# zgspose/PAVENet

Measured on AMD Instinct MI355X. Metric: clips/sec (T=7, 800x1344) fwd, higher is better.
Workload: dtype f32 (exact 3-term bf16 split on the bf16 MFMA)

## Files before the change

include/pave_hip.h:

```cpp
#ifndef PAVE_HIP_H_
#define PAVE_HIP_H_

#include <stdint.h>

#ifdef __cplusplus
extern "C" {
#endif

#define PAVE_OK 0
#define PAVE_E_ARG (-1)
#define PAVE_E_LAUNCH (-2)
#define PAVE_E_STEP (-3)
#define PAVE_E_UNSUPPORTED (-4)

#define PAVE_ABI_VERSION 21
int pave_abi_version(void);
const char* pave_last_error(void);

int pave_ms_deform_attn_forward_f32(const float* value, const int64_t* spatial_shapes,
                                    const int64_t* level_start, const float* sampling_loc,
                                    const float* attn_weight, float* out, int bs, int S, int M,
                                    int D, int L, int Lq, int P, int im2col_step, void* stream);
int pave_ms_deform_attn_forward_f64(const double* value, const int64_t* spatial_shapes,
                                    const int64_t* level_start, const double* sampling_loc,
// ... 648 lines not shown
                                 float* out, long long M, int K, int N, int group_n, int relu,
                                 int nplanes, void* stream);

int pave_gemm_bf16x3_ln_f32(const float* a, const void* w_planes, const float* bias,
                            const float* residual, const float* gamma, const float* beta, float eps,
                            float* out, long long M, int K, int N, int nplanes, void* stream);

int pave_conv3x3_split_f32(const float* x, const void* w_planes, const float* bias,
                           const float* residual, float* y, int N, int H, int W, int Cin, int Cout,
                           int stride, int relu, int nplanes, void* stream);

long long pave_conv3x3_splitk_workspace_bytes(int N, int H, int W, int Cin, int Cout, int stride);
int pave_conv3x3_splitk_f32(const float* x, const void* w_planes, const float* bias,
                            const float* residual, float* y, int N, int H, int W, int Cin, int Cout,
                            int stride, int relu, void* workspace, long long workspace_bytes,
                            int nplanes, void* stream);

long long pave_gemm_splitk_workspace_bytes(long long M, int K, int N);
int pave_gemm_bf16x3_splitk_f32(const float* a, const void* w_planes, const float* bias, const float* residual,
                                float* out, long long M, int K, int N, int relu, int nplanes, void* workspace,
                                long long workspace_bytes, void* stream);

int pave_set_form_policy(int policy);
int pave_get_form_policy(void);

#define PAVE_FORM_ROWS 0
#define PAVE_FORM_ROWS_SPLITK 1
#define PAVE_FORM_ROWS_TILE 2
#define PAVE_FORM_LN 3
#define PAVE_FORM_CONV3X3 4
#define PAVE_FORM_CONV1X1S 5
#define PAVE_FORM_ENCPROJ 6
#define PAVE_ORDER_TILE 0
#define PAVE_ORDER_KSPLIT 1
#define PAVE_ORDER_SPLITK 2
#define PAVE_ORDER_TILE_LNPASS 3
#define PAVE_ORDER_KSPLIT_LNPASS 4
#define PAVE_ORDER_TILE_LN8 5
int pave_form_plan(long long M, int K, int N, int kind, int nplanes, int policy, int* order, int* ksplit);

int pave_bottleneck_chain_f32(const float* c1, const void* w2_planes, const float* b2, float* c2,
                              const void* w3_planes, const float* b3, const float* residual,
                              const float* a2, int k2, float* out, const void* w1n_planes,
                              const float* b1n, float* c1n, int cn, int N, int H, int W, int nplanes,
                              void* stream);

int pave_conv1x1_strided_split_f32(const float* x, const void* w_planes, const float* bias, float* y,
                                   int N, int H, int W, int Cin, int Cout, int stride, int relu,
                                   int nplanes, void* stream);

int pave_conv7x7s2_nchw_split_f32(const float* x, const void* w_planes, const float* bias, float* y,
                                  int N, int H, int W, int row_pitch, int Cout, int relu, int nplanes,
                                  void* stream);

int pave_repitch_rows_f32(const float* src, float* dst, long long rows, int W, int pitch, void* stream);

int pave_swin_window_attn_f32(const float* qkv, const float* bias_t, const float* pad_qkv, float* out, int B,
                              int H, int W, int C, int heads, int window, int shift, float scale, void* stream);

int pave_merge_softmax_partials_f32(const float* parts, float* out, int G, int U, int C, int H, void* stream);

int pave_split_bf16x3_f32(const float* x, void* planes, long long n, int nplanes, void* stream);

#define PAVE_AUG_MAX_AUGS 16
#define PAVE_AUG_MAX_SLOTS 128
#define PAVE_AUG_MAX_K 64
typedef struct pave_aug_plan {
  const float* bboxes[PAVE_AUG_MAX_AUGS];
  const float* kpts[PAVE_AUG_MAX_AUGS];
  const int32_t* keep[PAVE_AUG_MAX_AUGS];
  int32_t flip[PAVE_AUG_MAX_AUGS];
  float img_w[PAVE_AUG_MAX_SLOTS];
  float scale_factor[PAVE_AUG_MAX_SLOTS][4];
  int32_t flip_perm[PAVE_AUG_MAX_K];
  int32_t n_aug, B, N, K;
} pave_aug_plan;
int pave_aug_merge_nms_f32(const pave_aug_plan* plan, float score_thr, int max_num, int method, float iou_thr,
                           float sigma, float min_score, int offset, float* dets, int64_t* labels, float* kpts,
                           int64_t* inds, int32_t* keep, int32_t* count, void* stream);

int pave_hflip_canvas_f32(const float* x, float* y, const int32_t* valid_w, int valid_w_all, int n, int C, int Hp,
                          int Wp, void* stream);

#ifdef __cplusplus
}
#endif
#endif
```

pavenet_amd/build_native.py:

```python
import os
import subprocess
import sysconfig

_HERE = os.path.dirname(os.path.abspath(__file__))
ROOT = os.path.dirname(_HERE)
SOURCES = [os.path.join(_HERE, 'csrc', 'pave_kernels.hip'),
           os.path.join(_HERE, 'csrc', 'pave_gemm_split.hip'),
           os.path.join(_HERE, 'csrc', 'pave_enc_tile.hip'),
           os.path.join(_HERE, 'csrc', 'pave_gemm_dma.hip'),
           os.path.join(_HERE, 'csrc', 'pave_decoder.hip'),
           os.path.join(_HERE, 'csrc', 'pave_aug.hip'),
           os.path.join(_HERE, 'csrc', 'pave_ingest.hip'),
           os.path.join(_HERE, 'csrc', 'pave_draw.hip'),
           os.path.join(_HERE, 'csrc', 'pave_track.hip'),
           os.path.join(_HERE, 'csrc', 'pave_smooth.hip'),
           os.path.join(_HERE, 'csrc', 'pave_zones.hip'),
           os.path.join(_HERE, 'csrc', 'pave_posture.hip'),
           os.path.join(_HERE, 'csrc', 'pave_overlay.hip'),
           os.path.join(_HERE, 'csrc', 'pave_heat.hip'),
           os.path.join(_HERE, 'csrc', 'pave_trails.hip'),
           os.path.join(_HERE, 'csrc', 'pave_floor.hip'),
           os.path.join(_HERE, 'csrc', 'pave_contacts.hip'),
           os.path.join(_HERE, 'csrc', 'pave_reid.hip'),
           os.path.join(_HERE, 'csrc', 'pave_anon.hip')]
HEADERS = sorted(os.path.join(_HERE, 'csrc', f) for f in os.listdir(os.path.join(_HERE, 'csrc')) if f.endswith('.h')) + \
          [os.path.join(ROOT, 'include', 'pave_hip.h')]
OUT = os.path.join(_HERE, 'lib', 'libpave_hip.so')
OUT_DIAG = os.path.join(_HERE, 'lib', 'libpave_hip_diag.so')
EXT_SOURCE = os.path.join(_HERE, 'csrc', 'pave_mmcv_ext.cpp')
EXT_OUT = os.path.join(_HERE, '_ext' + (sysconfig.get_config_var('EXT_SUFFIX') or '.so'))


def _fresh(out, deps):
    return os.path.exists(out) and all(os.path.getmtime(out) >= os.path.getmtime(s) for s in deps)


def build_native(force=False, verbose=False, diag=True):
    os.makedirs(os.path.dirname(OUT), exist_ok=True)
    flavours = [('', [], OUT)] + ([('_diag', ['-DPAVE_DIAG=1'], OUT_DIAG)] if diag else [])
    hipcc = os.environ.get('HIPCC', '/opt/rocm/bin/hipcc')
    procs, links = [], []
    for suffix, defs, out in flavours:
        if not force and _fresh(out, SOURCES + HEADERS):
            continue
        objs = []
        for src in SOURCES:
            obj = os.path.join(_HERE, 'lib', os.path.basename(src).replace('.hip', suffix + '.o'))
            objs.append(obj)
            if not force and _fresh(obj, [src] + HEADERS):
                continue
            cmd = [hipcc, '-O3', '--offload-arch=gfx950', '-std=c++17', '-fPIC', '-c'] + defs + \
                  ['-I' + os.path.join(ROOT, 'include'), '-o', obj, src]
            if verbose and not suffix:
                cmd.insert(1, '-Rpass-analysis=kernel-resource-usage')
            procs.append((cmd, subprocess.Popen(cmd)))
        links.append((out, objs))
    for cmd, p in procs:
        if p.wait() != 0:
            raise subprocess.CalledProcessError(p.returncode, cmd)
    for out, objs in links:
        subprocess.check_call([hipcc, '--offload-arch=gfx950', '-shared', '-fPIC', '-o', out] + objs)
    return OUT


def build_ext(force=False):
    if not force and _fresh(EXT_OUT, [EXT_SOURCE, OUT] + HEADERS):
        return EXT_OUT
    import torch
    from torch.utils.cpp_extension import include_paths, library_paths
    cmd = ['g++', '-O2', '-std=c++17', '-shared', '-fPIC', '-D__HIP_PLATFORM_AMD__=1', '-DUSE_ROCM=1',
           '-DTORCH_EXTENSION_NAME=_ext', '-DTORCH_API_INCLUDE_EXTENSION_H',
           f'-D_GLIBCXX_USE_CXX11_ABI={int(torch._C._GLIBCXX_USE_CXX11_ABI)}',
           '-I/opt/rocm/include', '-I' + os.path.join(ROOT, 'include'),
           '-I' + sysconfig.get_paths()['include']] + ['-I' + p for p in include_paths()] + \
          [EXT_SOURCE, '-o', EXT_OUT, '-L' + os.path.dirname(OUT), '-lpave_hip',
           '-Wl,-rpath,$ORIGIN/lib'] + \
          [a for p in library_paths() for a in ('-L' + p, '-Wl,-rpath,' + p)] + \
          ['-lc10', '-lc10_hip', '-ltorch_cpu', '-ltorch_hip', '-ltorch', '-ltorch_python']
    subprocess.check_call(cmd)
    return EXT_OUT


if __name__ == '__main__':
    print(build_native(force=True, verbose=True))
    print(build_ext(force=True))
```

pavenet_amd/deform_attn.py:

```python
import math
import warnings

import torch
import torch.nn as nn

from . import ops
from .bricks import (BaseModule, SourceKey, batch_first, constant_init, linear_residual_norm,
                     linear_rows, seq_first_view, xavier_init)
from .census import note_slow_path
from .registry import ATTENTION, MMCV_ATTENTION


def frame_prefixes(num_frames):
    assert num_frames % 2 == 1, 'num_frames must be odd (centre frame + symmetric neighbours)'
    c = num_frames // 2
    return ['pre_' * (c - t) if t < c else 'next_' * (t - c) for t in range(num_frames)]


def _check_heads(embed_dims, num_heads):
    if embed_dims % num_heads != 0:
        raise ValueError(f'embed_dims must be divisible by num_heads, '
                         f'but got {embed_dims} and {num_heads}')
    d = embed_dims // num_heads
    if not (isinstance(d, int) and d > 0 and (d & (d - 1)) == 0):
# ... 3 lines not shown


class _CatProj:

    def _cat_sources(self):
        raise NotImplementedError

    def _cat_proj(self, frames=None):
        offs, logits = self._cat_sources()
        if frames is not None:
            offs, logits = [offs[t] for t in frames], [logits[t] for t in frames]
        srcs = [m.weight for m in offs + logits] + [m.bias for m in offs + logits]
        key = SourceKey(srcs, frames)
        if getattr(self, '_cat_key', None) != key:
            with torch.no_grad():
                self._cat_w = torch.cat([m.weight for m in offs + logits], 0).contiguous()
                self._cat_b = torch.cat([m.bias for m in offs + logits], 0).contiguous()
            self._cat_key = key
        return self._cat_w, self._cat_b


FOLD_QUERY_POS = True


def cat_proj_rows(mod, query, query_pos, frames=None):
    from .bricks import fold_pos_ok, fused_mode
    q = batch_first(query)
    bs, Q, C = q.shape
    pos_rows = None
    if (FOLD_QUERY_POS and query_pos is not None and q.is_cuda and q.dtype == torch.float32 and fused_mode()
            and not torch.is_grad_enabled() and query_pos.shape == query.shape and C % 64 == 0 and q.is_contiguous()):
        pb = query_pos.transpose(0, 1)
        if fold_pos_ok(pb, bs) and pb.stride(2) == 1:
            pos_rows = pb[0]
    if pos_rows is None:
        w, b = mod._cat_proj(frames)
        if query_pos is not None:
            q = batch_first(query + query_pos)
        return linear_rows(q.reshape(bs * Q, C), w, b)
    w, b = mod._cat_proj(frames)
    base = pos_rows._base if pos_rows._base is not None else pos_rows
    from .bricks import get_gemm_mode
    key = SourceKey((base, w, b), extra=(tuple(pos_rows.shape), tuple(pos_rows.stride()), pos_rows.storage_offset(),
                                        frames, get_gemm_mode()))
    hit = mod.__dict__.get('_pave_pos_proj')
    if hit is None or hit[0] != key:
        with torch.no_grad():
            N = w.shape[0]
            Np = (N + 127) // 128 * 128
            wp = torch.zeros((Np, w.shape[1]), dtype=torch.float32, device=w.device)
            wp[:N] = w
            tab = torch.zeros((Q, Np), dtype=torch.float32, device=w.device)
            tab[:, :N] = (pos_rows.double() @ w.double().t() + b.double()).float()
            planes = ops.split_weight_bf16x3(wp, 3)
        hit = mod.__dict__['_pave_pos_proj'] = (key, planes, tab)
    return ops.gemm_bf16x3_ex(q.reshape(bs * Q, C), hit[1], None, hit[2], residual_rows=Q)[0]


def _proj(linear, x):
    if x.is_cuda and x.is_contiguous():
        y = linear_rows(x.reshape(-1, x.shape[-1]), linear.weight, linear.bias)
        return y.view(x.shape[:-1] + (y.shape[-1],))
    return linear(x)


PADDED_FAST_PATH = True


def masked_row_index(mask):
    base = mask._base if mask._base is not None else mask
    key = SourceKey((base,), (tuple(mask.shape), tuple(mask.stride()), mask.storage_offset()))
    slots = base.__dict__.setdefault('_pave_mask_rows', [])
    for k, idx in slots:
        if k == key:
            return idx
    with torch.no_grad():
        idx = mask.reshape(-1).nonzero().flatten().to(torch.int32)
    if len(slots) > 8:
        del slots[:]
    slots.append((key, idx))
    return idx


def project_values_hoisted(attns, value_bf, key_padding_mask=None, masked_rows=None):
    from .bricks import _split_weight, get_gemm_mode, split_gemm_ok
    x = value_bf
    fill = None
    if PADDED_FAST_PATH and key_padding_mask is not None and x.is_cuda and x.is_contiguous() and len(attns) >= 2 \
            and not torch.is_grad_enabled() and key_padding_mask.dtype == torch.bool \
            and all(type(a).project_value in (MulFramesMultiScaleDeformablePoseAttention.project_value,
                                              MulFramesMultiScaleDeformableAttention.project_value)
                    and a.value_proj.bias is not None for a in attns) \
            and split_gemm_ok(x.reshape(-1, x.shape[-1]), attns[0].value_proj.weight):
        fill = masked_rows if masked_rows is not None else masked_row_index(key_padding_mask)
        key_padding_mask = None
    if key_padding_mask is not None or not (x.is_cuda and x.is_contiguous()) or len(attns) < 2:
        return [a.project_value(value_bf, key_padding_mask) for a in attns]
    rows = x.reshape(-1, x.shape[-1])
    outs = []
    i = 0
    while i < len(attns):
        a = attns[i]
        b = attns[i + 1] if i + 1 < len(attns) else None
        if b is not None and a.value_proj.out_features == b.value_proj.out_features \
                and a.value_proj.out_features % 128 == 0 \
                and split_gemm_ok(rows, a.value_proj.weight):
            srcs = (a.value_proj.weight, a.value_proj.bias, b.value_proj.weight, b.value_proj.bias)
            key = SourceKey(srcs)
            if getattr(a, '_pair_key', None) != key:
                with torch.no_grad():
                    a._pair_w = torch.cat([a.value_proj.weight, b.value_proj.weight], 0).contiguous()
                    a._pair_b = torch.cat([a.value_proj.bias, b.value_proj.bias], 0).contiguous()
                a._pair_key = key
            nv = a.value_proj.out_features
            v1, v2 = ops.gemm_bf16x3_ex(rows, _split_weight(a._pair_w), a._pair_b, n_split=nv,
                                        fp16=get_gemm_mode() == 'fp16')
            for m, v in ((a, v1), (b, v2)):
                if fill is not None:
                    ops.fill_rows_(v, fill, m.value_proj.bias.detach())
                outs.append(v.view(-1, x.shape[-2], m.num_heads, nv // m.num_heads))
            i += 2
        else:
            v = a.project_value(value_bf, None)
            if fill is not None:
                ops.fill_rows_(v.view(-1, v.shape[-2] * v.shape[-1]), fill, a.value_proj.bias.detach())
            outs.append(v)
            i += 1
    return outs


def _fused_ok(mod, *tensors):
    return (mod.embed_dims == 256 and mod.num_heads == 8
            and all(t.is_cuda and t.dtype == torch.float32 for t in tensors))


def _host_levels(spatial_shapes, kwargs):
    hs = kwargs.get('spatial_shapes_host')
    if hs is not None:
        return [(int(h), int(w)) for h, w in hs]
    return [(int(h), int(w)) for h, w in spatial_shapes.tolist()]


@MMCV_ATTENTION.register_module()
class MultiScaleDeformableAttention(BaseModule, _CatProj):

    def __init__(self, embed_dims=256, num_heads=8, num_levels=4, num_points=4, im2col_step=64,
                 dropout=0.1, batch_first=False, norm_cfg=None, init_cfg=None):
        super().__init__(init_cfg)
        _check_heads(embed_dims, num_heads)
        self.norm_cfg = norm_cfg
        self.dropout = nn.Identity()
        self.batch_first = batch_first
        self.im2col_step = im2col_step
        self.prepare_in_gemm = True
        self.embed_dims = embed_dims
        self.num_levels = num_levels
        self.num_heads = num_heads
        self.num_points = num_points
        self.sampling_offsets = nn.Linear(embed_dims, num_heads * num_levels * num_points * 2)
        self.attention_weights = nn.Linear(embed_dims, num_heads * num_levels * num_points)
        self.value_proj = nn.Linear(embed_dims, embed_dims)
        self.output_proj = nn.Linear(embed_dims, embed_dims)
        self.init_weights()

    def init_weights(self):
        constant_init(self.sampling_offsets, 0.)
        thetas = torch.arange(self.num_heads, dtype=torch.float32) * (2.0 * math.pi / self.num_heads)
        grid_init = torch.stack([thetas.cos(), thetas.sin()], -1)
        grid_init = (grid_init / grid_init.abs().max(-1, keepdim=True)[0]).view(
            self.num_heads, 1, 1, 2).repeat(1, self.num_levels, self.num_points, 1)
        for i in range(self.num_points):
            grid_init[:, :, i, :] *= i + 1
        with torch.no_grad():
            self.sampling_offsets.bias.copy_(grid_init.view(-1))
        constant_init(self.attention_weights, val=0., bias=0.)
        xavier_init(self.value_proj, distribution='uniform', bias=0.)
        xavier_init(self.output_proj, distribution='uniform', bias=0.)
        self._is_init = True

    def _cat_sources(self):
        return [self.sampling_offsets], [self.attention_weights]

    supports_post_norm = True
    supports_query_plus_pos = True

    def _tile_shift(self):
        b = self.sampling_offsets.bias
        key = SourceKey((b,))
        if getattr(self, '_tile_shift_key', None) != key:
            self._tile_shift_val = ops.enc_tile_window_shift(b)
            self._tile_shift_key = key
        return self._tile_shift_val

    def _merged_proj(self):
        w_cat, b_cat = self._cat_proj()
        srcs = (self.value_proj.weight, self.value_proj.bias, w_cat, b_cat)
        key = SourceKey(srcs)
        if getattr(self, '_merged_key', None) != key:
            with torch.no_grad():
                self._merged_w = torch.cat([self.value_proj.weight, w_cat], 0).contiguous()
            self._merged_key = key
        return self._merged_w, w_cat, b_cat

    def _forward_merged(self, q, pos_row, reference_points, tile_levels, out_half=False):
        from .bricks import _split_weight, fused_mode, get_gemm_mode
        bs, S, C = q.shape
        w_all, w_cat, b_cat = self._merged_proj()
        nv = self.value_proj.out_features
        src = pos_row._base if pos_row._base is not None else pos_row
# ... 561 lines not shown
```

pavenet_amd/ops.py:

```python
import contextlib
import ctypes
import numbers

import torch

from . import native


KERNEL_EVENTS = None
KERNEL_EVENT_TAGS = ('enc_tile', 'enc_grid_T1')
KERNEL_EVENT_SHAPES = None


def _stream_ptr():
    return torch.cuda.current_stream().cuda_stream


FORM_ROWS, FORM_ROWS_SPLITK, FORM_ROWS_TILE, FORM_LN, FORM_CONV3X3, FORM_CONV1X1S, FORM_ENCPROJ = (
    native.DEFINES['PAVE_FORM_' + n] for n in ('ROWS', 'ROWS_SPLITK', 'ROWS_TILE', 'LN', 'CONV3X3', 'CONV1X1S',
                                               'ENCPROJ'))
ORDER_TILE, ORDER_KSPLIT, ORDER_SPLITK, ORDER_TILE_LNPASS, ORDER_KSPLIT_LNPASS, ORDER_TILE_LN8 = (
    native.DEFINES['PAVE_ORDER_' + n] for n in ('TILE', 'KSPLIT', 'SPLITK', 'TILE_LNPASS', 'KSPLIT_LNPASS',
                                                'TILE_LN8'))


def current_form_policy():
    return native.load().pave_get_form_policy()


@contextlib.contextmanager
def form_policy(p):
    _require(p in (0, 1, 2), 'form_policy: 0, 1 or 2')
    lib = native.load()
    prev = lib.pave_get_form_policy()
    native.check(lib.pave_set_form_policy(int(p)), 'set_form_policy')
    try:
        yield
    finally:
        lib.pave_set_form_policy(prev)


def form_plan(M, K, N, kind=FORM_ROWS, policy=None, planes=3):
    lib = native.load()
    order, parts = ctypes.c_int(), ctypes.c_int()
    st = lib.pave_form_plan(int(M), int(K), int(N), int(kind), 16 if planes == PLANES_FP16 else int(planes),
                            current_form_policy() if policy is None else int(policy), ctypes.byref(order),
                            ctypes.byref(parts))
    native.check(st, 'form_plan')
    return order.value, parts.value


class _Timed:
    def __init__(self, tag, flops=0, shape=None):
        self.tag = tag if (KERNEL_EVENTS is not None and tag in KERNEL_EVENT_TAGS) else None
        self.flops = flops
        if self.tag is not None and KERNEL_EVENT_SHAPES is not None:
            KERNEL_EVENT_SHAPES.append(shape)

    def __enter__(self):
        if self.tag is not None:
            self.s = torch.cuda.Event(enable_timing=True)
            self.e = torch.cuda.Event(enable_timing=True)
            self.s.record()

    def __exit__(self, *a):
        if self.tag is not None:
            self.e.record()
            KERNEL_EVENTS.append((self.tag, self.s, self.e, self.flops))


SMALL_ROWS = 8192


def _gemm_tag(tag, M):
    return tag if M >= SMALL_ROWS else tag + '_small'


def _require(cond, msg):
    if not cond:
        raise RuntimeError(msg)


def _dev(t, name, dtype=None):
    _require(isinstance(t, torch.Tensor), f'{name} must be a tensor')
    _require(t.is_cuda, f'{name} must be a HIP device tensor (pavenet_amd has no CPU path)')
    _require(t.is_contiguous(), f'{name} tensor has to be contiguous')
    if dtype is not None:
        _require(t.dtype == dtype, f'{name} must be {dtype}, got {t.dtype}')
    return t


def _nhwc(x, who):
    _require(x.is_cuda and x.dtype == torch.float32 and x.dim() == 4, f'{who}: fp32 4-D')
    _require(x.is_contiguous(memory_format=torch.channels_last), f'{who}: channels_last input')


def _ptr(t):
    return t.data_ptr() if t is not None else None


def _launch(entry, what, dev, *args, tag=None, flops=0, shape=None):
    fn = getattr(native.load(), entry)
    with torch.cuda.device(dev), _Timed(tag, flops, shape):
        st = fn(*args, _stream_ptr())
    native.check(st, what)


PLANES_FP16 = native.DEFINES['PAVE_PLANES_FP16']


def _planes(w_planes, name='w_planes', fp16=False, only=None):
    dt = w_planes.dtype if isinstance(w_planes, torch.Tensor) else None
    if not (dt in (torch.int16, torch.float16) and w_planes.is_cuda and w_planes.is_contiguous()
            and w_planes.dim() == 4 and w_planes.shape[3] == 16):
        _dev(w_planes, name)
        _require(dt in (torch.int16, torch.float16), f'{name} must be int16 (bf16 planes) or float16 (fp16 plane)')
        _require(False, f'{name}: [K/16, planes, N, 16] (split_weight_bf16x3)')
    n = w_planes.shape[1]
    if dt == torch.float16 or fp16:
        _require(n == 1, f'{name}: fp16 operands are a single plane')
        n = PLANES_FP16
    if only is not None and n not in only:
        _require(False, f'{name}: this entry point takes 3 bf16 planes or one fp16 plane')
    return n


_Q_PLANES = (3, PLANES_FP16)


def ms_deform_attn_forward(value, value_spatial_shapes, value_level_start_index,
                           sampling_locations, attention_weights, im2col_step=64):
    _require(value.dtype in (torch.float32, torch.float64),
             'ms_deform_attn_forward: value must be float32 or float64')
    dt = value.dtype
    _dev(value, 'value', dt)
    _dev(value_spatial_shapes, 'spatial_shapes', torch.int64)
    _dev(value_level_start_index, 'level_start_index', torch.int64)
    _dev(sampling_locations, 'sampling_loc', dt)
    _dev(attention_weights, 'attn_weight', dt)
    _require(value.dim() == 4 and sampling_locations.dim() == 6 and attention_weights.dim() == 5,
             'ms_deform_attn_forward: bad tensor ranks')
    bs, S, M, D = value.shape
    _, Lq, M2, L, P, two = sampling_locations.shape
    _require(M2 == M and two == 2 and sampling_locations.shape[0] == bs,
             'ms_deform_attn_forward: sampling_loc shape mismatch')
    _require(tuple(attention_weights.shape) == (bs, Lq, M, L, P),
             'ms_deform_attn_forward: attn_weight shape mismatch')
    _require(tuple(value_spatial_shapes.shape) == (L, 2) and
             tuple(value_level_start_index.shape) == (L,),
             'ms_deform_attn_forward: spatial_shapes / level_start_index shape mismatch')
    out = torch.empty((bs, Lq, M * D), dtype=dt, device=value.device)
    if out.numel() == 0:
        return out
    _launch('pave_ms_deform_attn_forward_f32' if dt == torch.float32 else 'pave_ms_deform_attn_forward_f64',
            'ms_deform_attn_forward', value.device,
            value.data_ptr(), value_spatial_shapes.data_ptr(),
            value_level_start_index.data_ptr(), sampling_locations.data_ptr(),
            attention_weights.data_ptr(), out.data_ptr(), bs, S, M, D, L, Lq, P,
            int(im2col_step))
    return out


def ms_deform_attn_backward(value, value_spatial_shapes, value_level_start_index,
                            sampling_locations, attention_weights, grad_output, grad_value,
                            grad_sampling_loc, grad_attn_weight, im2col_step=64):
    dt = value.dtype
    _require(dt in (torch.float32, torch.float64), 'ms_deform_attn_backward: fp32 / fp64 only')
    for t, n in ((value, 'value'), (sampling_locations, 'sampling_loc'),
                 (attention_weights, 'attn_weight'), (grad_output, 'grad_output'),
                 (grad_value, 'grad_value'), (grad_sampling_loc, 'grad_sampling_loc'),
                 (grad_attn_weight, 'grad_attn_weight')):
        _dev(t, n, dt)
    _dev(value_spatial_shapes, 'spatial_shapes', torch.int64)
    _dev(value_level_start_index, 'level_start_index', torch.int64)
    bs, S, M, D = value.shape
    _, Lq, _, L, P, _ = sampling_locations.shape
    _require(grad_output.numel() == bs * Lq * M * D and grad_value.shape == value.shape and
             grad_sampling_loc.shape == sampling_locations.shape and
             grad_attn_weight.shape == attention_weights.shape,
             'ms_deform_attn_backward: gradient shapes mismatch')
    if grad_output.numel() == 0:
        return
    _launch('pave_ms_deform_attn_backward_f32' if dt == torch.float32 else 'pave_ms_deform_attn_backward_f64',
            'ms_deform_attn_backward', value.device,
            value.data_ptr(), value_spatial_shapes.data_ptr(),
            value_level_start_index.data_ptr(), sampling_locations.data_ptr(),
            attention_weights.data_ptr(), grad_output.data_ptr(), grad_value.data_ptr(),
            grad_sampling_loc.data_ptr(), grad_attn_weight.data_ptr(), bs, S, M, D, L, Lq, P,
# ... 2389 lines not shown
```

pavenet_amd/transformer.py:

```python

import torch
import torch.nn as nn

from .bricks import (BaseModule, SourceKey, TransformerLayerSequence, batch_first, inverse_sigmoid,
                     linear_norm, mlp_rows, query_rows_scope,
                     seq_first_view, xavier_init)
from .deform_attn import (MulFramesMultiScaleDeformableAttention,
                          MulFramesMultiScaleDeformablePoseAttention,
                          MultiScaleDeformableAttention, frame_prefixes,
                          project_values_hoisted)
from .locality import encoder_unit_order
from .registry import (MMCV_TRANSFORMER, MMCV_TRANSFORMER_LAYER_SEQUENCE, TRANSFORMER,
                       TRANSFORMER_LAYER_SEQUENCE, build_transformer_layer_sequence)

_REF_BRANCH_KW = ('pre_pre_', 'pre_', '', 'next_', 'next_next_')


def _collect_frame_branches(T, kwargs, suffix):
    generic = kwargs.pop('frame_' + suffix, None)
    named = {p: kwargs.pop(p + suffix, None) for p in _REF_BRANCH_KW}
    if generic is not None:
        assert len(generic) == T
        return list(generic)
    if named[''] is None:
# ... 281 lines not shown
        return output, reference_points


@TRANSFORMER_LAYER_SEQUENCE.register_module()
class PetrTransformerDecoder(TransformerLayerSequence):

    def __init__(self, *args, return_intermediate=False, num_keypoints=17, **kwargs):
        super().__init__(*args, **kwargs)
        self.return_intermediate = return_intermediate
        self.num_keypoints = num_keypoints

    def forward(self, query, *args, reference_points=None, valid_ratios=None, kpt_branches=None,
                **kwargs):
        K = self.num_keypoints
        output = query
        intermediate, intermediate_reference_points = [], []
        for lid, layer in enumerate(self.layers):
            if reference_points.shape[-1] == K * 2:
                reference_points_input = reference_points[:, :, None] * \
                    valid_ratios.repeat(1, 1, K)[:, None]
            else:
                assert reference_points.shape[-1] == 2
                reference_points_input = reference_points[:, :, None] * valid_ratios[:, None]
            output = layer(output, *args, reference_points=reference_points_input, **kwargs)
            output = output.permute(1, 0, 2)
            if kpt_branches is not None:
                tmp = mlp_rows(kpt_branches[lid], output)
                if reference_points.shape[-1] == K * 2:
                    reference_points = (tmp + inverse_sigmoid(reference_points)).sigmoid().detach()
                else:
                    raise NotImplementedError
            output = output.permute(1, 0, 2)
            if self.return_intermediate:
                intermediate.append(output)
                intermediate_reference_points.append(reference_points)
        if self.return_intermediate:
            return torch.stack(intermediate), torch.stack(intermediate_reference_points)
        return output, reference_points


@MMCV_TRANSFORMER.register_module()
class Transformer(BaseModule):

    def __init__(self, encoder=None, decoder=None, init_cfg=None):
        super().__init__(init_cfg=init_cfg)
        self.encoder = build_transformer_layer_sequence(encoder)
        self.decoder = build_transformer_layer_sequence(decoder)
        self.embed_dims = self.encoder.embed_dims

    def init_weights(self):
        for m in self.modules():
            if hasattr(m, 'weight') and m.weight is not None and m.weight.dim() > 1:
                xavier_init(m, distribution='uniform')
        self._is_init = True


UNIT_ORDER_MODE = 'band'


class _LevelGeometry:

    def __init__(self, hw_list, device):
        self.hw = [(int(h), int(w)) for h, w in hw_list]
        self.spatial_shapes = torch.as_tensor(self.hw, dtype=torch.long, device=device)
        starts = [0]
        for h, w in self.hw[:-1]:
            starts.append(starts[-1] + h * w)
        self.starts = starts
        self.level_start_index = torch.as_tensor(starts, dtype=torch.long, device=device)
        self.S = sum(h * w for h, w in self.hw)
        self._order = {}
        self.unpadded = {}

    def unit_order(self, n_frames, device):
        if n_frames not in self._order:
            self._order[n_frames] = encoder_unit_order(self.hw, n_frames, UNIT_ORDER_MODE).to(device)
        return self._order[n_frames]

    def tile_levels(self):
        from .ops import enc_tile_supported
        return self.hw if enc_tile_supported(self.hw) else None


@TRANSFORMER.register_module()
class VideoPoseTransformerMulFrames(Transformer):

    def __init__(self, hm_encoder=None, refine_decoder=None, as_two_stage=True,
                 num_feature_levels=4, two_stage_num_proposals=300, num_keypoints=17,
                 num_frames=3, **kwargs):
        super().__init__(**kwargs)
        self.as_two_stage = as_two_stage
        self.num_feature_levels = num_feature_levels
        self.two_stage_num_proposals = two_stage_num_proposals
        self.embed_dims = self.encoder.embed_dims
        self.num_keypoints = num_keypoints
        self.num_frames = num_frames
        self.refine_decoder = build_transformer_layer_sequence(refine_decoder)
        self.init_layers()
        self._geom = {}
        self.hoist_value_proj = True
        self.xcd_unit_order = True
        self.enc_lds_tile = True
        self.fused_proposal_stage = True

    def init_layers(self):
        self.level_embeds = nn.Parameter(torch.Tensor(self.num_feature_levels, self.embed_dims))
        if self.as_two_stage:
            self.enc_output = nn.Linear(self.embed_dims, self.embed_dims)
            self.enc_output_norm = nn.LayerNorm(self.embed_dims)
            self.refine_query_embedding = nn.Embedding(self.num_keypoints, self.embed_dims * 2)
        else:
            self.reference_points = nn.Linear(self.embed_dims, 2 * self.num_keypoints)

    def init_weights(self):
        for p in self.parameters():
            if p.dim() > 1:
                nn.init.xavier_uniform_(p)
        for m in self.modules():
            if isinstance(m, MultiScaleDeformableAttention):
                m.init_weights()
        if not self.as_two_stage:
            xavier_init(self.reference_points, distribution='uniform', bias=0.)
        nn.init.normal_(self.level_embeds)
        nn.init.normal_(self.refine_query_embedding.weight)
        self._is_init = True

    def geometry(self, hw_list, device):
        key = (tuple((int(h), int(w)) for h, w in hw_list), str(device))
        if key not in self._geom:
            self._geom[key] = _LevelGeometry(hw_list, device)
        return self._geom[key]

    def gen_encoder_output_proposals(self, memory, memory_padding_mask, geom, mask_key=None):
        N, S, C = memory.shape
        dev = memory.device
        cached = None
        if memory_padding_mask is None and memory.is_cuda and not torch.is_grad_enabled():
            cached = geom.unpadded.get(('proposals', N))
            if cached is not None:
                output_proposals, valid = cached
                filled = self._output_memory_filled(memory, valid, geom) if self.fused_proposal_stage else None
                if filled is not None:
                    return filled, output_proposals
                output_memory = memory.masked_fill(~valid, float(0))
                output_memory = linear_norm(output_memory, self.enc_output, self.enc_output_norm)
                return output_memory, output_proposals
        if memory_padding_mask is not None and mask_key is not None and memory.is_cuda \
                and not torch.is_grad_enabled() and self.fused_proposal_stage:
            hit = geom.unpadded.get(('proposals_padded', N))
            if hit is not None and hit[0] == mask_key:
                _, output_proposals, keep = hit
                filled = self._output_memory_filled(memory, keep, geom, tag=('padded', N), key_extra=mask_key)
                if filled is not None:
                    return filled, output_proposals
        proposals = []
        _cur = 0
        for lvl, (H, W) in enumerate(geom.hw):
            if memory_padding_mask is not None:
                m = memory_padding_mask[:, _cur:(_cur + H * W)].view(N, H, W, 1)
                valid_H = torch.sum(~m[:, :, 0, 0], 1)
                valid_W = torch.sum(~m[:, 0, :, 0], 1)
            else:
                valid_H = torch.full((N,), H, device=dev)
                valid_W = torch.full((N,), W, device=dev)
            grid_y, grid_x = torch.meshgrid(
                torch.linspace(0, H - 1, H, dtype=torch.float32, device=dev),
                torch.linspace(0, W - 1, W, dtype=torch.float32, device=dev), indexing='ij')
            grid = torch.cat([grid_x.unsqueeze(-1), grid_y.unsqueeze(-1)], -1)
            scale = torch.cat([valid_W.unsqueeze(-1), valid_H.unsqueeze(-1)], 1).view(N, 1, 1, 2)
            grid = (grid.unsqueeze(0).expand(N, -1, -1, -1) + 0.5) / scale
            proposals.append(grid.view(N, -1, 2))
            _cur += H * W
        output_proposals = torch.cat(proposals, 1)
        valid = ((output_proposals > 0.01) & (output_proposals < 0.99)).all(-1, keepdim=True)
        output_proposals = torch.log(output_proposals / (1 - output_proposals))
        if memory_padding_mask is not None:
            output_proposals = output_proposals.masked_fill(
                memory_padding_mask.unsqueeze(-1), float('inf'))
        output_proposals = output_proposals.masked_fill(~valid, float('inf'))
        if memory_padding_mask is None and memory.is_cuda and not torch.is_grad_enabled():
            geom.unpadded[('proposals', N)] = (output_proposals, valid)
            filled = self._output_memory_filled(memory, valid, geom) if self.fused_proposal_stage else None
            if filled is not None:
# ... 71 lines not shown
    def _frame_branch_lists(self, kwargs, suffix):
        return _collect_frame_branches(self.num_frames, kwargs, suffix)

    @staticmethod
    def _flat_view(mlvl_feats):
        f0 = mlvl_feats[0]
        n, C = f0.shape[:2]
        S = sum(f.shape[2] * f.shape[3] for f in mlvl_feats)
        off = 0
        for f in mlvl_feats:
            h, w = f.shape[2:]
            if f.dtype != f0.dtype or f.stride() != (S * C, 1, w * C, C) or \
                    f.data_ptr() != f0.data_ptr() + off * C * f0.element_size():
                return None
            off += h * w
        return f0.as_strided((n, S, C), (S * C, C, 1))

    def encode_frames(self, mlvl_feats, mlvl_masks, mlvl_pos_embeds, has_padding=True):
        dev = mlvl_feats[0].device
        geom = self.geometry([f.shape[-2:] for f in mlvl_feats], dev)
        feat_flatten = [feat.flatten(2).transpose(1, 2) for feat in mlvl_feats]
        flat = self._flat_view(mlvl_feats) if feat_flatten[0].is_cuda else None
        feat_flatten = flat if flat is not None else torch.cat(feat_flatten, 1)
        key = SourceKey(list(mlvl_masks) + list(mlvl_pos_embeds) + [self.level_embeds])
        const = geom.unpadded.get('flat_pos') if (feat_flatten.is_cuda
                                                   and not torch.is_grad_enabled()) else None
        if const is not None and const[0] == key:
            mask_flatten, lvl_pos_embed_flatten = const[1], const[2]
        else:
            mask_flatten, lvl_pos_embed_flatten = [], []
            for lvl, (mask, pos_embed) in enumerate(zip(mlvl_masks, mlvl_pos_embeds)):
                mask_flatten.append(mask.flatten(1))
                pos_embed = pos_embed.flatten(2).transpose(1, 2)
                lvl_pos_embed_flatten.append(pos_embed + self.level_embeds[lvl].view(1, 1, -1))
            mask_flatten = torch.cat(mask_flatten, 1)
            lvl_pos_embed_flatten = torch.cat(lvl_pos_embed_flatten, 1)
            if feat_flatten.is_cuda and not torch.is_grad_enabled():
                geom.unpadded['flat_pos'] = (key, mask_flatten, lvl_pos_embed_flatten)
        if lvl_pos_embed_flatten.shape[0] != feat_flatten.shape[0]:
            lvl_pos_embed_flatten = lvl_pos_embed_flatten.expand(feat_flatten.shape[0], -1, -1)
        spatial_shapes, level_start_index = geom.spatial_shapes, geom.level_start_index
        nfr = feat_flatten.shape[0]
        const = geom.unpadded.get(('refs', nfr)) if (not has_padding and feat_flatten.is_cuda) else None
        if const is not None:
            valid_ratios, reference_points = const
        else:
            pkey = SourceKey(list(mlvl_masks), extra=nfr)
            phit = geom.unpadded.get(('refs_padded', nfr)) if (feat_flatten.is_cuda
                                                               and not torch.is_grad_enabled()) else None
            if phit is not None and phit[0] == pkey:
                valid_ratios, reference_points = phit[1], phit[2]
            else:
                valid_ratios = torch.stack([self.get_valid_ratio(m) for m in mlvl_masks], 1)
                if valid_ratios.shape[0] != nfr:
                    valid_ratios = valid_ratios.expand(nfr, -1, -1)
                reference_points = self.get_reference_points(geom.hw, valid_ratios, device=dev)
                if feat_flatten.is_cuda and not torch.is_grad_enabled():
                    if has_padding:
                        geom.unpadded[('refs_padded', nfr)] = (pkey, valid_ratios, reference_points)
                    else:
                        geom.unpadded[('refs', nfr)] = (valid_ratios.contiguous(), reference_points)
        attn_mask = mask_flatten if has_padding else None
        if attn_mask is not None and attn_mask.shape[0] != feat_flatten.shape[0]:
            attn_mask = attn_mask.expand(feat_flatten.shape[0], -1)
        bs = feat_flatten.shape[0]
        extra = {}
        if self.enc_lds_tile and feat_flatten.is_cuda and geom.tile_levels() is not None:
            extra['tile_levels'] = geom.tile_levels()
            groups = getattr(mlvl_masks, 'frame_groups', None)
            if attn_mask is not None and groups is not None and sum(n for _, n in groups) == bs:
                extra['frame_groups'] = groups
                extra['masked_rows'] = mlvl_masks.masked_rows()
        elif self.xcd_unit_order and feat_flatten.is_cuda:
            extra['unit_order'] = geom.unit_order(bs, dev)
        extra['inplace_residual'] = True
        extra['input_is_shared'] = flat is not None
        memory = self.encoder(
            query=seq_first_view(feat_flatten), key=None, value=None,
            query_pos=seq_first_view(lvl_pos_embed_flatten), query_key_padding_mask=attn_mask,
            spatial_shapes=spatial_shapes, reference_points=reference_points,
            level_start_index=level_start_index, valid_ratios=valid_ratios, **extra)
        return batch_first(memory), mask_flatten, valid_ratios, geom

    def forward(self, mlvl_feats, mlvl_masks, query_embed, mlvl_pos_embeds, cls_branches=None,
                sigma_branches=None, has_padding=True, frame_shard=None, **kwargs):
        assert self.as_two_stage or query_embed is not None
        T = self.num_frames
        Tl = T if frame_shard is None else frame_shard.n_local
        branches = self._frame_branch_lists(kwargs, 'kpt_branches')
        kpt_branches = branches[T // 2] if branches is not None else None
        encoded = kwargs.pop('encoded', None)
        if encoded is None:
            encoded = self.encode_frames(mlvl_feats, mlvl_masks, mlvl_pos_embeds, has_padding)
        memory, mask_flatten, valid_ratios, geom = encoded
        dev = memory.device
        bs = memory.shape[0]
        spatial_shapes, level_start_index = geom.spatial_shapes, geom.level_start_index
        attn_mask = mask_flatten if has_padding else None
        if attn_mask is not None and attn_mask.shape[0] != bs:
            attn_mask = attn_mask.expand(bs, -1)
        c = memory.shape[-1]
        n_clips = bs // Tl
        if frame_shard is None:
            ctr = slice(T // 2, None, T)
        elif frame_shard.owns_center():
            ctr = slice(frame_shard.local_index_of_center(), None, Tl)
        else:
            ctr = slice(0, None, Tl)
        now_frame_memory = memory[ctr]
        now_frame_mask_flatten = mask_flatten[ctr] if mask_flatten.shape[0] == bs else mask_flatten
        now_frame_valid_ratios = valid_ratios[ctr]
        if self.as_two_stage:
            mask_key = SourceKey((mask_flatten,), extra=(ctr.start, ctr.step, now_frame_memory.shape[0])) \
                if (has_padding and frame_shard is None) else None
            output_memory, output_proposals = self.gen_encoder_output_proposals(
                now_frame_memory, now_frame_mask_flatten if has_padding else None, geom, mask_key=mask_key)
            enc_outputs_class = mlp_rows(cls_branches[self.decoder.num_layers], output_memory)
            topk = self.two_stage_num_proposals
            logits = enc_outputs_class[..., 0]
            if (logits.is_cuda and logits.dtype == torch.float32 and logits.shape[1] <= 32768
                    and topk <= 1024 and not torch.is_grad_enabled()):
                from . import ops
                topk_proposals = ops.topk_rows(logits, topk)[1]
            else:
                topk_proposals = torch.topk(logits, topk, dim=1)[1]
            forced = kwargs.pop('force_topk_proposals', None)
            if forced is not None:
                topk_proposals = forced
            self.last_topk_proposals = topk_proposals
            self.last_enc_cls = enc_outputs_class
            query_pos, query = torch.split(query_embed, c, dim=1)
            fused = (self.fused_proposal_stage and output_memory.is_cuda
                     and output_memory.dtype == torch.float32 and frame_shard is None
                     and not torch.is_grad_enabled() and output_memory.is_contiguous() and c % 4 == 0
                     and output_proposals.is_contiguous())
            fused_query = None
            if fused:
                from . import ops
                topk_proposals = topk_proposals.contiguous()
                tgt, fused_query = ops.gather_rows_add(output_memory, topk_proposals,
                                                       self._dense_const('query_half', query_embed, query))
            else:
                tgt = torch.gather(output_memory, 1,
                                   topk_proposals.unsqueeze(-1).repeat(1, 1, self.embed_dims))
            with query_rows_scope():
                topk_kpts_unact = mlp_rows(kpt_branches[self.decoder.num_layers], tgt)
            fused_refs = None
            if fused and topk_kpts_unact.stride(-1) == 1:
                fused_refs = ops.proposal_refs_(topk_kpts_unact, output_proposals, topk_proposals, T)
            else:
                top_props = torch.gather(output_proposals, 1,
                                         topk_proposals.unsqueeze(-1).repeat(1, 1, 2))
                topk_kpts_unact[..., 0::2] += top_props[..., 0:1]
                topk_kpts_unact[..., 1::2] += top_props[..., 1:2]
            enc_outputs_kpt_unact = topk_kpts_unact
            with query_rows_scope():
                enc_outputs_sigma_unact = mlp_rows(sigma_branches[self.decoder.num_layers], tgt)
            if frame_shard is not None:
                from . import dist as pdist
                tgt, topk_kpts_unact = tgt.contiguous(), topk_kpts_unact.contiguous()
                enc_outputs_kpt_unact = topk_kpts_unact
                enc_outputs_sigma_unact = enc_outputs_sigma_unact.contiguous()
                for t_ in (tgt, topk_kpts_unact, enc_outputs_sigma_unact):
                    pdist.broadcast_from(t_, frame_shard.center_owner, frame_shard.group)
            reference_points = fused_refs if fused_refs is not None else \
                topk_kpts_unact.sigmoid().repeat(1, T, 1)
            init_reference_out = reference_points
            query_pos = query_pos.unsqueeze(0).expand(n_clips, -1, -1)
            query = fused_query if fused_query is not None else \
                tgt + query.unsqueeze(0).expand(n_clips, -1, -1)
        else:
            query_pos, query = torch.split(query_embed, c, dim=1)
            query_pos = query_pos.unsqueeze(0).expand(bs, -1, -1)
            query = query.unsqueeze(0).expand(bs, -1, -1)
            reference_points = self.reference_points(query_pos).sigmoid()
            init_reference_out = reference_points
            enc_outputs_class = enc_outputs_kpt_unact = enc_outputs_sigma_unact = None
        dec_kwargs = {}
        if branches is not None:
            dec_kwargs['frame_kpt_branches'] = branches
        if frame_shard is not None:
            dec_kwargs['frame_shard'] = frame_shard
        if not has_padding and isinstance(self.decoder, VideoPoseTransformerDecoderMulFrames):
            dec_kwargs['unit_valid_ratios'] = True
        cached = kwargs.pop('values_projected', None)
        if cached is not None:
            dec_kwargs['values_projected'] = cached
            dec_kwargs['value_frame_table'] = kwargs.pop('value_frame_table')
        elif self.hoist_value_proj and all(
                isinstance(l.attentions[-1], MulFramesMultiScaleDeformablePoseAttention)
                for l in self.decoder.layers):
            dec_kwargs['values_projected'] = project_values_hoisted(
                [l.attentions[-1] for l in self.decoder.layers], memory, attn_mask,
                masked_rows=mlvl_masks.masked_rows() if (attn_mask is not None
                                                         and hasattr(mlvl_masks, 'masked_rows')) else None)
        with query_rows_scope():
            inter_states, inter_references = self.decoder(
                query=seq_first_view(query.contiguous()), key=None, value=seq_first_view(memory),
                query_pos=seq_first_view(query_pos), key_padding_mask=attn_mask,
                reference_points=reference_points, spatial_shapes=spatial_shapes,
                level_start_index=level_start_index, valid_ratios=now_frame_valid_ratios,
                **dec_kwargs)
        memory_out = seq_first_view(memory)
        if self.as_two_stage:
            return inter_states, init_reference_out, inter_references, enc_outputs_class, \
                enc_outputs_kpt_unact, enc_outputs_sigma_unact, None, memory_out
        return inter_states, init_reference_out, inter_references, None, None, None, None, None, None

    def forward_refine(self, mlvl_masks, memory, reference_points_pose, img_inds,
                       has_padding=True, frame_shard=None, **kwargs):
        T = self.num_frames
        Tl = T if frame_shard is None else frame_shard.n_local
        branches = self._frame_branch_lists(kwargs, 'kpt_branches')
        dev = memory.device
        geom = self.geometry([m.shape[-2:] for m in mlvl_masks], dev)
        spatial_shapes, level_start_index = geom.spatial_shapes, geom.level_start_index
        const = geom.unpadded.get(('refine', mlvl_masks[0].shape[0])) \
            if (not has_padding and memory.is_cuda) else None
        pkey = SourceKey(list(mlvl_masks)) if (has_padding and memory.is_cuda and not torch.is_grad_enabled()) else None
        phit = geom.unpadded.get(('refine_padded', mlvl_masks[0].shape[0])) if pkey is not None else None
        if const is not None:
            mask_flatten, valid_ratios = const
        elif phit is not None and phit[0] == pkey:
            mask_flatten, valid_ratios = phit[1], phit[2]
        else:
            mask_flatten = torch.cat([m.flatten(1) for m in mlvl_masks], 1)
            valid_ratios = torch.stack([self.get_valid_ratio(m) for m in mlvl_masks], 1)
            if not has_padding and memory.is_cuda and not torch.is_grad_enabled():
                geom.unpadded[('refine', mlvl_masks[0].shape[0])] = (mask_flatten, valid_ratios)
            elif pkey is not None:
                geom.unpadded[('refine_padded', mlvl_masks[0].shape[0])] = (pkey, mask_flatten, valid_ratios)
        B = memory.shape[1]
        if valid_ratios.shape[0] != B * Tl:
            valid_ratios = valid_ratios.expand(B * Tl, -1, -1)
            mask_flatten = mask_flatten.expand(B * Tl, -1)
        rq = self.refine_query_embedding.weight
        query_pos, query = torch.split(rq, rq.size(1) // 2, dim=1)
        pos_num = reference_points_pose.size(0) // T
        query_pos = query_pos.unsqueeze(0).expand(pos_num, -1, -1)
        query = query.unsqueeze(0).expand(pos_num, -1, -1)
        if query.is_cuda and not torch.is_grad_enabled():
            query = self._dense_const('refine_query', rq, query, rows=pos_num)
        reference_points = reference_points_pose.reshape(-1, reference_points_pose.size(1) // 2, 2)
        mask_bt = mask_flatten.reshape(-1, Tl, mask_flatten.size(-1))
        if has_padding:
            vkey = SourceKey((valid_ratios, img_inds), extra=(Tl, T, frame_shard is not None)) if pkey is not None else None
            vhit = self.__dict__.get('_pave_vr_rows')
            if vkey is not None and vhit is not None and vhit[0] == vkey:
                vr_rows = vhit[1]
            else:
                vr = valid_ratios.reshape(-1, Tl, valid_ratios.size(-2), valid_ratios.size(-1))[img_inds]
                if frame_shard is not None:
                    vr = vr[:, :1].expand(-1, T, -1, -1)
                vr_rows = vr.transpose(0, 1).flatten(0, 1)
                if vkey is not None:
                    self.__dict__['_pave_vr_rows'] = (vkey, vr_rows)
        else:
            vr_rows = valid_ratios[:1].expand(img_inds.shape[0] * T, -1, -1)
        dec_kwargs = {}
        if branches is not None:
            dec_kwargs['frame_reg_branches'] = branches
        if frame_shard is not None:
            dec_kwargs['frame_shard'] = frame_shard
        if not has_padding and isinstance(self.refine_decoder, DeformableDetrTransformerDecoderMulFrames):
            dec_kwargs['unit_valid_ratios'] = True
        mem_bt = memory.permute(1, 2, 0, 3)
        attn_mask = mask_bt if has_padding else None
        cached = kwargs.pop('values_projected', None)
        if cached is not None:
            dec_kwargs['values_projected'] = cached
            dec_kwargs['value_frame_table'] = kwargs.pop('value_frame_table')
        elif self.hoist_value_proj and all(
                isinstance(l.attentions[-1], MulFramesMultiScaleDeformableAttention)
                for l in self.refine_decoder.layers):
            dec_kwargs['values_projected'] = project_values_hoisted(
                [l.attentions[-1] for l in self.refine_decoder.layers], mem_bt, attn_mask,
                masked_rows=mlvl_masks.masked_rows() if (attn_mask is not None
                                                         and hasattr(mlvl_masks, 'masked_rows')) else None)
        with query_rows_scope():
            inter_states, inter_references = self.refine_decoder(
                query=seq_first_view(query.contiguous()), key=None, value=memory,
                query_pos=seq_first_view(query_pos), key_padding_mask=attn_mask,
                reference_points=reference_points, spatial_shapes=spatial_shapes,
                level_start_index=level_start_index, valid_ratios=vr_rows,
                memory_clip_index=img_inds, **dec_kwargs)
        return inter_states, reference_points, inter_references
```

Baseline: 59.38.

## Run hoisted decoder value projections on a low-priority side stream

Adds a native side-queue module with per-device low-priority streams and fork/mark/join events. The hoisted value projections for both the pose decoder and the refine decoder are issued on the side stream right after the encoder, so they can overlap with proposal/query-prep work on the main stream. Each decoder layer's values are wrapped so that the first access joins on the matching event. This adds event and ctypes overhead and cross-stream memory-lifetime handling via record_stream, and it falls back to the caller stream under graph capture or when grad is enabled.

```diff
diff --git a/include/pave_hip.h b/include/pave_hip.h
--- a/include/pave_hip.h
+++ b/include/pave_hip.h
@@ -754,6 +754,14 @@
 int pave_hflip_canvas_f32(const float* x, float* y, const int32_t* valid_w, int valid_w_all, int n, int C, int Hp,
                           int Wp, void* stream);
 
+#define PAVE_SIDE_SLOTS 4
+#define PAVE_SIDE_MAX_QUEUES 2
+int pave_side_queue_get(void** stream, int* priority);
+int pave_side_queue_fork(void* caller_stream, int* on_side, void** stream);
+int pave_side_queue_mark(int slot);
+int pave_side_queue_join(void* caller_stream, int slot);
+int pave_side_queue_count(void);
+
 #ifdef __cplusplus
 }
 #endif
diff --git a/pavenet_amd/build_native.py b/pavenet_amd/build_native.py
--- a/pavenet_amd/build_native.py
+++ b/pavenet_amd/build_native.py
@@ -22,7 +22,8 @@
            os.path.join(_HERE, 'csrc', 'pave_floor.hip'),
            os.path.join(_HERE, 'csrc', 'pave_contacts.hip'),
            os.path.join(_HERE, 'csrc', 'pave_reid.hip'),
-           os.path.join(_HERE, 'csrc', 'pave_anon.hip')]
+           os.path.join(_HERE, 'csrc', 'pave_anon.hip'),
+           os.path.join(_HERE, 'csrc', 'pave_side_queue.hip')]
 HEADERS = sorted(os.path.join(_HERE, 'csrc', f) for f in os.listdir(os.path.join(_HERE, 'csrc')) if f.endswith('.h')) + \
           [os.path.join(ROOT, 'include', 'pave_hip.h')]
 OUT = os.path.join(_HERE, 'lib', 'libpave_hip.so')
diff --git a/pavenet_amd/csrc/pave_side_queue.hip b/pavenet_amd/csrc/pave_side_queue.hip
--- /dev/null
+++ b/pavenet_amd/csrc/pave_side_queue.hip
@@ -0,0 +1,148 @@
+#include <hip/hip_runtime.h>
+
+#include <cstdio>
+#include <mutex>
+
+#include "pave_hip.h"
+#include "pave_internal.h"
+
+namespace {
+
+struct SideQueue {
+  int device = -1;
+  int priority = 0;
+  hipStream_t stream = nullptr;
+  hipEvent_t forked = nullptr;
+  hipEvent_t ready[PAVE_SIDE_SLOTS] = {};
+  bool marked[PAVE_SIDE_SLOTS] = {};
+};
+
+std::mutex g_mu;
+SideQueue g_queues[PAVE_SIDE_MAX_QUEUES];
+int g_nqueues = 0;
+
+int hip_fail(const char* what, hipError_t e) {
+  (void)hipGetLastError();
+  static thread_local char msg[160];
+  snprintf(msg, sizeof(msg), "%s: %s", what, hipGetErrorString(e));
+  return pave_internal_fail(PAVE_E_LAUNCH, msg);
+}
+
+SideQueue* find_or_create(bool create, int* st) {
+  *st = PAVE_OK;
+  int dev = -1;
+  hipError_t e = hipGetDevice(&dev);
+  if (e != hipSuccess) {
+    *st = hip_fail("side queue: hipGetDevice", e);
+    return nullptr;
+  }
+  for (int i = 0; i < g_nqueues; ++i)
+    if (g_queues[i].device == dev) return &g_queues[i];
+  if (!create) return nullptr;
+  if (g_nqueues >= PAVE_SIDE_MAX_QUEUES) {
+    *st = pave_internal_fail(PAVE_E_UNSUPPORTED, "side queue: this process already owns its two side streams");
+    return nullptr;
+  }
+  SideQueue q;
+  q.device = dev;
+  int least = 0, greatest = 0;
+  if ((e = hipDeviceGetStreamPriorityRange(&least, &greatest)) != hipSuccess) {
+    *st = hip_fail("side queue: hipDeviceGetStreamPriorityRange", e);
+    return nullptr;
+  }
+  q.priority = least;
+  if ((e = hipStreamCreateWithPriority(&q.stream, hipStreamNonBlocking, least)) != hipSuccess) {
+    *st = hip_fail("side queue: hipStreamCreateWithPriority", e);
+    return nullptr;
+  }
+  e = hipEventCreateWithFlags(&q.forked, hipEventDisableTiming);
+  for (int s = 0; s < PAVE_SIDE_SLOTS && e == hipSuccess; ++s)
+    e = hipEventCreateWithFlags(&q.ready[s], hipEventDisableTiming);
+  if (e != hipSuccess) {
+    if (q.forked) (void)hipEventDestroy(q.forked);
+    for (int s = 0; s < PAVE_SIDE_SLOTS; ++s)
+      if (q.ready[s]) (void)hipEventDestroy(q.ready[s]);
+    (void)hipStreamDestroy(q.stream);
+    *st = hip_fail("side queue: hipEventCreateWithFlags", e);
+    return nullptr;
+  }
+  g_queues[g_nqueues] = q;
+  return &g_queues[g_nqueues++];
+}
+
+bool capturing(hipStream_t s, int* st) {
+  hipStreamCaptureStatus cs = hipStreamCaptureStatusNone;
+  const hipError_t e = hipStreamIsCapturing(s, &cs);
+  if (e != hipSuccess) {
+    *st = hip_fail("side queue: hipStreamIsCapturing", e);
+    return true;
+  }
+  return cs != hipStreamCaptureStatusNone;
+}
+
+}
+
+extern "C" int pave_side_queue_count(void) {
+  std::lock_guard<std::mutex> lock(g_mu);
+  return g_nqueues;
+}
+
+extern "C" int pave_side_queue_get(void** stream, int* priority) {
+  if (!stream) return pave_internal_fail(PAVE_E_ARG, "side queue: stream is null");
+  std::lock_guard<std::mutex> lock(g_mu);
+  int st;
+  SideQueue* q = find_or_create(true, &st);
+  if (!q) return st;
+  *stream = (void*)q->stream;
+  if (priority) *priority = q->priority;
+  return PAVE_OK;
+}
+
+extern "C" int pave_side_queue_fork(void* caller_stream, int* on_side, void** stream) {
+  if (!on_side || !stream) return pave_internal_fail(PAVE_E_ARG, "side queue: on_side / stream is null");
+  *on_side = 0;
+  *stream = caller_stream;
+  hipStream_t caller = (hipStream_t)caller_stream;
+  std::lock_guard<std::mutex> lock(g_mu);
+  int st = PAVE_OK;
+  if (capturing(caller, &st)) return st;
+  SideQueue* q = find_or_create(true, &st);
+  if (!q) return st == PAVE_E_UNSUPPORTED ? PAVE_OK : st;
+  if (caller == q->stream) return PAVE_OK;
+  hipError_t e = hipEventRecord(q->forked, caller);
+  if (e != hipSuccess) return hip_fail("side queue: hipEventRecord(fork)", e);
+  if ((e = hipStreamWaitEvent(q->stream, q->forked, 0)) != hipSuccess)
+    return hip_fail("side queue: hipStreamWaitEvent(fork)", e);
+  *on_side = 1;
+  *stream = (void*)q->stream;
+  return PAVE_OK;
+}
+
+extern "C" int pave_side_queue_mark(int slot) {
+  if (slot < 0 || slot >= PAVE_SIDE_SLOTS) return pave_internal_fail(PAVE_E_ARG, "side queue: slot out of range");
+  std::lock_guard<std::mutex> lock(g_mu);
+  int st;
+  SideQueue* q = find_or_create(false, &st);
+  if (!q) return st != PAVE_OK ? st : pave_internal_fail(PAVE_E_ARG, "side queue: mark before fork");
+  const hipError_t e = hipEventRecord(q->ready[slot], q->stream);
+  if (e != hipSuccess) return hip_fail("side queue: hipEventRecord(mark)", e);
+  q->marked[slot] = true;
+  return PAVE_OK;
+}
+
+extern "C" int pave_side_queue_join(void* caller_stream, int slot) {
+  if (slot < 0 || slot >= PAVE_SIDE_SLOTS) return pave_internal_fail(PAVE_E_ARG, "side queue: slot out of range");
+  hipStream_t caller = (hipStream_t)caller_stream;
+  std::lock_guard<std::mutex> lock(g_mu);
+  int st;
+  SideQueue* q = find_or_create(false, &st);
+  if (!q) return st != PAVE_OK ? st : pave_internal_fail(PAVE_E_ARG, "side queue: join before fork");
+  if (!q->marked[slot]) return pave_internal_fail(PAVE_E_ARG, "side queue: join of a slot that was not marked");
+  if (caller == q->stream) return PAVE_OK;
+  st = PAVE_OK;
+  if (capturing(caller, &st))
+    return st != PAVE_OK ? st : pave_internal_fail(PAVE_E_ARG, "side queue: join inside a capture");
+  const hipError_t e = hipStreamWaitEvent(caller, q->ready[slot], 0);
+  if (e != hipSuccess) return hip_fail("side queue: hipStreamWaitEvent(join)", e);
+  return PAVE_OK;
+}
diff --git a/pavenet_amd/deform_attn.py b/pavenet_amd/deform_attn.py
--- a/pavenet_amd/deform_attn.py
+++ b/pavenet_amd/deform_attn.py
@@ -109,7 +109,7 @@
     return idx
 
 
-def project_values_hoisted(attns, value_bf, key_padding_mask=None, masked_rows=None):
+def project_values_hoisted(attns, value_bf, key_padding_mask=None, masked_rows=None, on_ready=None):
     from .bricks import _split_weight, get_gemm_mode, split_gemm_ok
     x = value_bf
     fill = None
@@ -122,7 +122,10 @@
         fill = masked_rows if masked_rows is not None else masked_row_index(key_padding_mask)
         key_padding_mask = None
     if key_padding_mask is not None or not (x.is_cuda and x.is_contiguous()) or len(attns) < 2:
-        return [a.project_value(value_bf, key_padding_mask) for a in attns]
+        outs = [a.project_value(value_bf, key_padding_mask) for a in attns]
+        if on_ready is not None:
+            on_ready(0, outs)
+        return outs
     rows = x.reshape(-1, x.shape[-1])
     outs = []
     i = 0
@@ -146,12 +149,16 @@
                 if fill is not None:
                     ops.fill_rows_(v, fill, m.value_proj.bias.detach())
                 outs.append(v.view(-1, x.shape[-2], m.num_heads, nv // m.num_heads))
+            if on_ready is not None:
+                on_ready(i, outs[i:])
             i += 2
         else:
             v = a.project_value(value_bf, None)
             if fill is not None:
                 ops.fill_rows_(v.view(-1, v.shape[-2] * v.shape[-1]), fill, a.value_proj.bias.detach())
             outs.append(v)
+            if on_ready is not None:
+                on_ready(i, outs[i:])
             i += 1
     return outs
 
diff --git a/pavenet_amd/ops.py b/pavenet_amd/ops.py
--- a/pavenet_amd/ops.py
+++ b/pavenet_amd/ops.py
@@ -104,6 +104,63 @@
     with torch.cuda.device(dev), _Timed(tag, flops, shape):
         st = fn(*args, _stream_ptr())
     native.check(st, what)
+
+
+SIDE_SLOTS = native.DEFINES['PAVE_SIDE_SLOTS']
+
+
+class SideQueue:
+
+    def __init__(self, device, inputs=()):
+        self.device = torch.device(device)
+        lib = self._lib = native.load()
+        on_side, stream = ctypes.c_int(0), ctypes.c_void_p()
+        with torch.cuda.device(self.device):
+            self.caller = torch.cuda.current_stream()
+            native.check(lib.pave_side_queue_fork(self.caller.cuda_stream, ctypes.byref(on_side),
+                                                  ctypes.byref(stream)), 'side_queue_fork')
+        self.on_side = bool(on_side.value)
+        self.stream = torch.cuda.ExternalStream(stream.value, device=self.device) if self.on_side else self.caller
+        self._scope = None
+        self._joined = set()
+        if self.on_side:
+            for t in inputs:
+                t.record_stream(self.stream)
+
+    def __enter__(self):
+        if self.on_side:
+            self._scope = torch.cuda.stream(self.stream)
+            self._scope.__enter__()
+        return self
+
+    def __exit__(self, *exc):
+        if self._scope is not None:
+            scope, self._scope = self._scope, None
+            return scope.__exit__(*exc)
+
+    def mark(self, slot, *outputs):
+        _require(0 <= slot < SIDE_SLOTS, f'side queue: slot in [0, {SIDE_SLOTS})')
+        if not self.on_side:
+            return
+        with torch.cuda.device(self.device):
+            native.check(self._lib.pave_side_queue_mark(int(slot)), 'side_queue_mark')
+        for t in outputs:
+            t.record_stream(self.caller)
+
+    def join(self, slot):
+        if not self.on_side or slot in self._joined:
+            return
+        with torch.cuda.device(self.device):
+            native.check(self._lib.pave_side_queue_join(self.caller.cuda_stream, int(slot)), 'side_queue_join')
+        self._joined.add(slot)
+
+
+def side_queue_info(device=None):
+    lib = native.load()
+    stream, prio = ctypes.c_void_p(), ctypes.c_int()
+    with torch.cuda.device(device):
+        native.check(lib.pave_side_queue_get(ctypes.byref(stream), ctypes.byref(prio)), 'side_queue_get')
+    return stream.value, prio.value, lib.pave_side_queue_count()
 
 
 PLANES_FP16 = native.DEFINES['PAVE_PLANES_FP16']
diff --git a/pavenet_amd/transformer.py b/pavenet_amd/transformer.py
--- a/pavenet_amd/transformer.py
+++ b/pavenet_amd/transformer.py
@@ -387,6 +387,19 @@
         return self.hw if enc_tile_supported(self.hw) else None
 
 
+class _SideValues:
+
+    def __init__(self, side, values, slots):
+        self.side, self.values, self.slots = side, values, slots
+
+    def __len__(self):
+        return len(self.values)
+
+    def __getitem__(self, lid):
+        self.side.join(self.slots[lid])
+        return self.values[lid]
+
+
 @TRANSFORMER.register_module()
 class VideoPoseTransformerMulFrames(Transformer):
 
@@ -404,6 +417,8 @@
         self.init_layers()
         self._geom = {}
         self.hoist_value_proj = True
+        self.side_value_proj = True
+        self.last_value_proj_stream = None
         self.xcd_unit_order = True
         self.enc_lds_tile = True
         self.fused_proposal_stage = True
@@ -641,6 +656,52 @@
             level_start_index=level_start_index, valid_ratios=valid_ratios, **extra)
         return batch_first(memory), mask_flatten, valid_ratios, geom
 
+    def _fork_value_proj(self, memory, attn_mask, mlvl_masks, n_clips):
+        self.__dict__.pop('_pave_side_refine', None)
+        self.last_value_proj_stream = 'caller'
+        pose = [l.attentions[-1] for l in self.decoder.layers]
+        joint = [l.attentions[-1] for l in self.refine_decoder.layers]
+        if not (self.side_value_proj and self.hoist_value_proj and memory.is_cuda and memory.is_contiguous()
+                and not torch.is_grad_enabled()
+                and all(isinstance(a, MulFramesMultiScaleDeformablePoseAttention) for a in pose)
+                and all(isinstance(a, MulFramesMultiScaleDeformableAttention) for a in joint)):
+            return None
+        from . import ops
+        side = ops.SideQueue(memory.device, inputs=(memory,))
+        if not side.on_side:
+            return None
+        T = self.num_frames
+        rows = mlvl_masks.masked_rows() if (attn_mask is not None and hasattr(mlvl_masks, 'masked_rows')) else None
+        slots, n_marks = {}, [0]
+
+        def ready(which):
+            def mark(first, tensors):
+                slot = min(n_marks[0], ops.SIDE_SLOTS - 1)
+                n_marks[0] += 1
+                side.mark(slot, *tensors)
+                for i in range(len(tensors)):
+                    slots[(which, first + i)] = slot
+            return mark
+        with side:
+            v_pose = project_values_hoisted(pose, memory, attn_mask, masked_rows=rows, on_ready=ready('pose'))
+            mem_bt = memory.view(n_clips, T, memory.shape[1], memory.shape[2])
+            mask_bt = attn_mask.reshape(n_clips, T, -1) if attn_mask is not None else None
+            v_joint = project_values_hoisted(joint, mem_bt, mask_bt, masked_rows=rows, on_ready=ready('joint'))
+        self.last_value_proj_stream = 'side'
+        self.__dict__['_pave_side_refine'] = (memory, memory._version, mlvl_masks, attn_mask is not None, _SideValues(
+            side, v_joint, [slots[('joint', i)] for i in range(len(joint))]))
+        return _SideValues(side, v_pose, [slots[('pose', i)] for i in range(len(pose))])
+
+    def _take_side_refine(self, mem_bt, mlvl_masks, has_padding):
+        hit = self.__dict__.pop('_pave_side_refine', None)
+        if hit is None:
+            return None
+        memory, version, masks, padded, values = hit
+        if (mem_bt.data_ptr() == memory.data_ptr() and mem_bt.numel() == memory.numel() and mem_bt.is_contiguous()
+                and mem_bt._version == version and masks is mlvl_masks and padded == bool(has_padding)):
+            return values
+        return None
+
     def forward(self, mlvl_feats, mlvl_masks, query_embed, mlvl_pos_embeds, cls_branches=None,
                 sigma_branches=None, has_padding=True, frame_shard=None, **kwargs):
         assert self.as_two_stage or query_embed is not None
@@ -660,6 +721,12 @@
             attn_mask = attn_mask.expand(bs, -1)
         c = memory.shape[-1]
         n_clips = bs // Tl
+        side_values = None
+        if frame_shard is None and 'values_projected' not in kwargs:
+            side_values = self._fork_value_proj(memory, attn_mask, mlvl_masks, n_clips)
+        else:
+            self.__dict__.pop('_pave_side_refine', None)
+            self.last_value_proj_stream = 'caller'
         if frame_shard is None:
             ctr = slice(T // 2, None, T)
         elif frame_shard.owns_center():
@@ -746,6 +813,8 @@
         if cached is not None:
             dec_kwargs['values_projected'] = cached
             dec_kwargs['value_frame_table'] = kwargs.pop('value_frame_table')
+        elif side_values is not None:
+            dec_kwargs['values_projected'] = side_values
         elif self.hoist_value_proj and all(
                 isinstance(l.attentions[-1], MulFramesMultiScaleDeformablePoseAttention)
                 for l in self.decoder.layers):
@@ -826,9 +895,14 @@
         mem_bt = memory.permute(1, 2, 0, 3)
         attn_mask = mask_bt if has_padding else None
         cached = kwargs.pop('values_projected', None)
+        side_values = self._take_side_refine(mem_bt, mlvl_masks, has_padding)
+        if cached is not None or frame_shard is not None:
+            side_values = None
         if cached is not None:
             dec_kwargs['values_projected'] = cached
             dec_kwargs['value_frame_table'] = kwargs.pop('value_frame_table')
+        elif side_values is not None:
+            dec_kwargs['values_projected'] = side_values
         elif self.hoist_value_proj and all(
                 isinstance(l.attentions[-1], MulFramesMultiScaleDeformableAttention)
                 for l in self.refine_decoder.layers):
```

Result: slower. 58.65 (-1.2%).
